# nilsbore/gp_compressor

Hardware: AMD Instinct MI355X
Metric: patches/sec (compress+predict) (higher is better)
Workload: dtype f64; 1 GPU; C2 room scan: 8192 patches x 256 pts per GPU, RBF + Gaussian noise, dense Cholesky fit + predictive mean on the 20x20 grid (m=400); patches_per_gpu=8192, points_per_patch=256, grid_points=400, parallelism=1 GPU, kernel=dense_mfma_w1

## Files before the change

gp_compressor_amd/capi.py:

```python
import ctypes as C
import os
import weakref

import numpy as np

HERE = os.path.dirname(os.path.abspath(__file__))
LIB_PATH = os.environ.get("GPC_LIB_PATH", os.path.join(HERE, "libgpc_hip.so"))

GPC_OK, GPC_EINVAL, GPC_ENOMEM, GPC_ENODEV, GPC_EHIP, GPC_ERANGE = 0, -22, -12, -19, -5, -34
CELL_UNOBSERVED, CELL_OCCUPIED, CELL_FREE = 0, 1, 2
STATUS_OK, STATUS_NOT_SPD, STATUS_NAN, STATUS_SIGMA_CLAMPED, STATUS_OVERFLOW, STATUS_NOT_CONVERGED = 0, 1, 2, 3, 4, 5
MAX_POINTS, MAX_BV = 1024, 256

c_dp = C.POINTER(C.c_double)
c_ip = C.POINTER(C.c_int32)


class Params(C.Structure):
    _fields_ = [("sigmaf_sq", C.c_double), ("l_sq", C.c_double), ("noise", C.c_double), ("eps_tol", C.c_double),
                ("capacity", C.c_int32), ("noise_model", C.c_int32), ("ref_double_noise", C.c_int32),
                ("ref_field_delete_bug", C.c_int32), ("want_variance", C.c_int32), ("reserved", C.c_int32)]


class IrlsParams(C.Structure):
# ... 151 lines not shown
    "gpc_comm_destroy": (None, [_vp]),
    "gpc_comm_world": (C.c_int, [_vp]),
    "gpc_comm_rank": (C.c_int, [_vp]),
    "gpc_comm_library": (C.c_char_p, []),
    "gpc_comm_set_partition": (C.c_int, [_vp, _i, _vp]),
    "gpc_group_start": (C.c_int, []),
    "gpc_group_end": (C.c_int, []),
    "gpc_allgather_fstar_dev": (C.c_int, [_vp, _i, _vp, _vp, _vp]),
    "gpc_unpermute_fstar_dev": (C.c_int, [_vp, _i, _vp, _vp]),
    "gpc_test_exp_host": (None, [_vp, _vp, _i]),
    "gpc_test_exp_small_host": (None, [_vp, _vp, _i]),
    "gpc_test_quantize_host": (C.c_int, [_vp, _i, _i, _vp, _vp, _vp]),
    "gpc_test_rate_allocate_host": (C.c_int, [_i, _i, _vp, _vp, _vp, _vp, _d, _vp, _i, C.c_int64, _i, _vp, _vp, _vp, _vp]),
    "gpc_test_par_memcpy": (None, [_vp, _vp, C.c_size_t]),
    "gpc_test_dense_route": (C.c_int, [_i] * 11 + [_vp, _i, _vp]),
}

_lib = None


def load():
    global _lib
    if _lib is not None:
        return _lib
    try:
        import torch
    except ImportError:
        pass
    if not os.path.exists(LIB_PATH):
        raise GpcError(GPC_ENODEV, f"{LIB_PATH} not built: run `python -c 'import __graft_entry__ as g; g.build()'` "
# ... 1261 lines not shown
    R, ld = a[2].shape
    k = np.zeros(R, dtype=np.int32)
    tg = None if count is None else np.zeros(R, dtype=np.int32)
    res = np.zeros(1, dtype=RATE_RESULT_DTYPE)
    rc = load().gpc_test_rate_allocate_host(R, ld, _ptr(a[0]), _ptr(a[1]), _ptr(a[2]), _ptr(a[3]), float(w_all), _ptr(a[4]), int(unit_all),
                                            int(need), int(bool(refine)), _ptr(a[5]), _ptr(k), _ptr(tg), _ptr(res))
    if rc != GPC_OK:
        raise GpcError(rc, "gpc_test_rate_allocate_host")
    return (k, rate_result(res)) if count is None else (k, tg, rate_result(res))


test_rate_allocate_host.__test__ = False


ROUTE_KINDS = {-1: "no route", 0: "nothing", 1: "one-wave", 2: "register", 3: "tiled", 4: "generic", 5: "split"}
ROUTE_SHAPE = ("w1_npad", "w1_slots", "nt", "export_factor", "waves", "npad", "per_cu", "nt17", "need_big")


def dense_route(P, n_max, n_total=None, ny=1, m=16, variance=False, pointwise=False, alpha_out=False, num_cus=256, irls=False,
                w1_refused=False):
    name = C.create_string_buffer(96)
    shape = np.zeros(len(ROUTE_SHAPE), dtype=np.int32)
    kind = load().gpc_test_dense_route(P, n_max, P * n_max if n_total is None else n_total, ny, m, int(variance), int(pointwise),
                                       int(alpha_out), num_cus, int(irls), int(w1_refused), name, len(name), _ptr(shape))
    return ROUTE_KINDS[kind], name.value.decode(), dict(zip(ROUTE_SHAPE, shape.tolist()))
```

gp_compressor_amd/csrc/dense_api.hip:

```cpp
#include "dense_internal.h"

int dense_check(gpc_ctx* ctx, const gpc_params* prm, int P, const void* off, int n_max, int n_total,
                const void* x0, const void* x1, const void* y, int ny, int m, const void* f_star)
{
    if (!ctx || ctx->dead.load()) return GPC_EINVAL;
    if (!prm) return gpc_fail(ctx, GPC_EINVAL, "params is NULL");
    if (P < 0 || m < 0 || n_total < 0 || n_max < 0) return gpc_fail(ctx, GPC_EINVAL, "negative size");
    if (ny != 1 && ny != 3) return gpc_fail(ctx, GPC_EINVAL, "ny must be 1 (depth) or 3 (RGB), got %d", ny);
    if (P > 0 && !off) return gpc_fail(ctx, GPC_EINVAL, "off is NULL");
    if (n_total > 0 && (!x0 || !x1 || !y)) return gpc_fail(ctx, GPC_EINVAL, "x0/x1/y is NULL");
    if (P > 0 && m > 0 && !f_star) return gpc_fail(ctx, GPC_EINVAL, "f_star is NULL");
    if (n_max > GPC_MAX_POINTS) return gpc_fail(ctx, GPC_ERANGE, "n_max %d > GPC_MAX_POINTS %d", n_max, GPC_MAX_POINTS);
    if (!(prm->l_sq > 0.0) || !(prm->sigmaf_sq >= 0.0) || !(prm->noise >= 0.0))
        return gpc_fail(ctx, GPC_EINVAL, "kernel/noise parameters out of range");
    return GPC_OK;
}

DenseArgs dense_args(const gpc_params* prm, int P, const int32_t* off, int n_max, int n_total, const double* x0, const double* x1,
                     const double* y, int ny, int m, double* f_star, double* alpha_out, int32_t* status)
{
    DenseArgs a{};
    a.prm = *prm;
    a.P = P; a.n_max = n_max; a.n_total = n_total; a.ny = ny; a.m = m;
    a.off = off; a.x0 = x0; a.x1 = x1; a.y = y;
// ... 83 lines not shown

int dense_dispatch(gpc_ctx* ctx, DenseArgs& a, const DenseSite& site, unsigned* seen_gen)
{
    const DenseSwitches sw = dense_switches_read();
    const DenseFacts facts = dense_facts(ctx, a);
    DenseRoute route = dense_route(facts, sw);
    if (route.kind == DENSE_NOTHING) return GPC_OK;
    if (a.n_max < 1) a.n_max = 1;
    if (seen_gen)
        if (int rco = gpc_pipe_chunk_order(ctx, site.stream, seen_gen)) return rco;
    GPC_HIP(ctx, hipSetDevice(ctx->device));
    if (!a.prm.want_variance) a.v_star = nullptr;
    if (int rcp = gpc_debug_poison_lds(ctx, site)) return rcp;
    int grid = 0, rc = GPC_OK;
    if (route.kind == DENSE_ONE_WAVE) {
        for (int cap_w1 = site.w1_cap;;) {
            rc = gpc_ws_reserve(ctx, site, al256(dense_w1_ws_bytes(facts, route, &grid, cap_w1)));
            if (rc != GPC_ENOMEM) break;
            cap_w1 = grid / 2;
            if (cap_w1 < 4 * ctx->num_cus) break;
        }
        if (rc == GPC_ENOMEM) {
            route = dense_route(facts, sw, true);
            if (route.kind == DENSE_NO_ROUTE) return rc;
            (void)hipGetLastError();
        } else if (rc != GPC_OK) {
            return rc;
        }
    }
    switch (route.kind) {
        case DENSE_ONE_WAVE:
            rc = dense_w1_launch(ctx, site, a, route, grid);
            break;
        case DENSE_REGISTER:
            rc = dense_mfma_launch(ctx, site, a, route);
            break;
        case DENSE_TILED:
            if ((rc = gpc_ws_reserve(ctx, site, al256(dense_big_ws_bytes(ctx, a, route, &grid)))) == GPC_OK)
                rc = dense_big_launch(ctx, site, a, route, grid);
            break;
        case DENSE_SPLIT:
            rc = dense_split(ctx, a, site, route, sw.no_hint);
            break;
// ... 13 lines not shown
    *w1_cap = 0;
    const DenseFacts facts = dense_facts(ctx, a);
    const DenseRoute route = dense_route(facts, dense_switches_read());
    int grid = 0, rc = GPC_ENOMEM;
    switch (route.kind) {
        case DENSE_NOTHING:
            return gpc_ws_reserve(ctx, site, front);
        case DENSE_ONE_WAVE:
            for (int cap_w1 = 0;;) {
                rc = gpc_ws_reserve(ctx, site, front + al256(dense_w1_ws_bytes(facts, route, &grid, cap_w1)));
                *w1_cap = cap_w1;
                if (rc != GPC_ENOMEM) break;
                cap_w1 = grid / 2;
                if (cap_w1 < 4 * ctx->num_cus) break;
            }
            return rc;
        case DENSE_REGISTER:
            return gpc_ws_reserve(ctx, site, front + dense_mfma_ws_bytes(a, route));
        case DENSE_TILED:
            return gpc_ws_reserve(ctx, site, front + al256(dense_big_ws_bytes(ctx, a, route, &grid)));
        case DENSE_GENERIC:
            return gpc_ws_reserve(ctx, site, front + dense_generic_ws_bytes(ctx, a, &grid));
        case DENSE_NO_ROUTE:
            return gpc_fail(ctx, GPC_ENOMEM, "no kernel computes the variance of this batch without the one-wave workspace");
        default:
            return gpc_fail(ctx, GPC_EINVAL, "dense_reserve: not a batch of the variance route");
    }
}

extern "C" {
// ... 22 lines not shown
    if (rc != GPC_OK) return rc;
    DenseArgs a = dense_args(params, P, off, n_max, n_total, x0, x1, y, ny, sz * sz, f_star, alpha_out, status);
    a.prm.want_variance = 0;
    a.grid_res = res; a.grid_sz = sz;
    std::lock_guard<std::mutex> lk(ctx->mu);
    return dense_dispatch(ctx, a, dense_site_of(ctx));
}

int gpc_test_dense_route(int P, int n_max, int n_total, int ny, int m, int variance, int pointwise, int alpha_out, int num_cus, int irls,
                         int w1_refused, char* name, int name_cap, int32_t* shape)
{
    const DenseFacts f{P, n_max, n_total, ny, m, variance != 0, pointwise != 0, alpha_out != 0, num_cus, irls != 0};
    const DenseRoute r = dense_route(f, dense_switches_read(), w1_refused != 0);
    if (name && name_cap > 0) snprintf(name, (size_t)name_cap, "%s", r.name);
    if (shape) {
        const int32_t v[GPC_TEST_ROUTE_SHAPE] = {r.w1_npad, r.w1_slots, r.nt, r.export_factor, r.waves, r.npad, r.per_cu, r.nt17, r.need_big};
        memcpy(shape, v, sizeof(v));
    }
    return (int)r.kind;
}

}
```

gp_compressor_amd/csrc/dense_mfma_w1.hip:

```cpp
#include <cstdio>
#include <cstdlib>
#include <type_traits>

#include "gpc_device.h"
#include "dense_internal.h"
#include "mfma_tile.h"

#define W1_NPAD_MAX 512
#define W1_C 4
#define W1_NDT 10
#define W1_NT_OF(npad) ((npad) / 16)
#define W1_TRI_OF(npad) (W1_NT_OF(npad) * (W1_NT_OF(npad) + 1) / 2)
#define W1_TILE(i, j) (((size_t)(i) * (size_t)((i) + 1) / 2 + (size_t)(j)) * MF_IMG)
#define W1_PACK_OF(npad) ((npad) <= 256)
#define W1_LNV_OF(npad) (W1_PACK_OF(npad) ? W1_NT_OF(npad) / 2 : W1_NT_OF(npad))


struct W1Params {
    DenseArgs a;
    double c_exp;
    double pivot_tol;
    double cs, noise_u, sfp, a_out;
    double* ws;
    double* linvt;
    int export_factor;
    unsigned long long* stamps;
};
#define W1_NPH 12
#ifdef W1_STAMPS
#define W1_STAMP(ph)                                                                                                 \
    do {                                                                                                             \
        __builtin_amdgcn_sched_barrier(0);                                                                           \
        const unsigned long long t_now_ = __builtin_amdgcn_s_memtime();                                              \
        st_acc_[ph] += t_now_ - t_prev_;                                                                             \
        t_prev_ = t_now_;                                                                                            \
        __builtin_amdgcn_sched_barrier(0);                                                                           \
    } while (0)
#else
#define W1_STAMP(ph) do { } while (0)
#endif
// ... 29 lines not shown
__device__ static __forceinline__ d4 w1_mfma4_neg(d4 a, d4 b, d4 acc)
{
#pragma unroll
    for (int s = 0; s < 4; ++s) acc = __builtin_amdgcn_mfma_f64_16x16x4f64(a[s], b[s], acc, 0, 0, 1);
    return acc;
}
__device__ static __forceinline__ d4 w1_trsm(d4 lv, d4 src)
{
    const d4 z4 = d4{0.0, 0.0, 0.0, 0.0};
    d4 D = __builtin_amdgcn_mfma_f64_16x16x4f64(lv[0], src[0], z4, 0, 0, 0);
    D = __builtin_amdgcn_mfma_f64_16x16x4f64(lv[1], src[1], D, 0, 0, 0);
    D = __builtin_amdgcn_mfma_f64_16x16x4f64(lv[2], src[2], D, 0, 0, 0);
    return __builtin_amdgcn_mfma_f64_16x16x4f64(lv[3], src[3], D, 0, 0, 0);
}

template <int MODE, int CNT, bool DIAG>
__device__ static __forceinline__ void w1_gram_row(d4 (&v)[W1_C], const double* px0, const double* px1, const double* T, double sf, bool scale_sf,
                                                   double cexp, double noise, bool dbl, int n, int r, int c0, int lr, int lg)
{
    const int pi = MF_TS * r + lr;
    const double xi0 = px0[pi], xi1 = px1[pi];
#pragma unroll
    for (int t = 0; t < CNT; ++t) {
#pragma unroll
        for (int q = 0; q < 4; ++q) {
            const int pj = MF_TS * (c0 + t) + lg + 4 * q;
            const double d0 = xi0 - px0[pj], d1 = xi1 - px1[pj];
            const double sq = __builtin_fma(d0, d0, d1 * d1);
            v[t][q] = MODE == 0 ? gpc_exp_neg(cexp * sq, T) : gpc_expm_poly<MODE == 1 ? 7 : 5>(sq);
        }
// ... 23 lines not shown
        }
    }
}

template <int W1_NPAD>
__global__ __launch_bounds__(64, 2) void dense_w1_kernel(W1Params g)
{
    constexpr int W1_NT = W1_NT_OF(W1_NPAD), W1_TRI = W1_TRI_OF(W1_NPAD);
    __shared__ __attribute__((aligned(16))) double T[GPC_EXP_TABLE_SIZE];
    __shared__ __attribute__((aligned(16))) double px0[W1_NPAD], px1[W1_NPAD], zv[W1_NPAD];
    __shared__ __attribute__((aligned(16))) double rsbuf[32], wsc[32];
    __shared__ __attribute__((aligned(16))) double LinvC[W1_C * MF_IMG];
    constexpr bool W1_PACK = W1_PACK_OF(W1_NPAD);
    constexpr int W1_LNV = W1_LNV_OF(W1_NPAD);
    __shared__ __attribute__((aligned(16))) double dgl[W1_PACK ? W1_LNV * MF_TS : 2];

    const DenseArgs& A = g.a;
    int lane = threadIdx.x;
    int lr = lane & 15, lg = lane >> 4;
#define W1_FRESH_LANE()                                                                                              \
    do {                                                                                                             \
        lane = mf_opaque(lane);                                                                                      \
        lr = lane & 15;                                                                                              \
        lg = lane >> 4;                                                                                              \
    } while (0)
    const int m = A.m;
    const double sf = A.prm.sigmaf_sq, cexp = g.c_exp;
    const bool dbl = A.prm.ref_double_noise != 0;
    const int patch = blockIdx.x;
    double* Lt = g.ws + (size_t)patch * W1_TRI * MF_IMG;
    double* LinvTg = g.linvt + (size_t)patch * W1_LNV * MF_IMG;

    gpc_exp_table_init(T);
    {
        const int o = __builtin_amdgcn_readfirstlane(A.off[patch]);
        const int n = __builtin_amdgcn_readfirstlane(A.off[patch + 1]) - o;
        double* fs = A.f_star + (size_t)patch * m;
        __syncthreads();
        if (n <= 0 || n > W1_NPAD) {
            for (int p = lane; p < m; p += 64) fs[p] = (n == 0) ? 0.0 : __builtin_nan("");
            if (lane == 0 && A.status) A.status[patch] = (n == 0) ? GPC_STATUS_OK : GPC_STATUS_NAN;
            return;
        }
        const int nt = __builtin_amdgcn_readfirstlane((n + MF_TS - 1) / MF_TS);
#ifdef W1_STAMPS
        unsigned long long st_acc_[W1_NPH] = {};
        unsigned long long t_prev_ = __builtin_amdgcn_s_memtime();
#endif

        const double xo0 = A.x0[o], xo1 = A.x1[o];
        double qr0[W1_NPAD / 64], qr1[W1_NPAD / 64];
        double mn0 = xo0, mx0 = xo0, mn1 = xo1, mx1 = xo1;
#pragma unroll
        for (int u = 0; u < W1_NPAD / 64; ++u) {
            const int i = lane + 64 * u;
            const bool live = i < n;
// ... 327 lines not shown
                    }
                    W1_STAMP(7);
                }
            }
            __syncthreads();
            W1_STAMP(8);
        }
#undef W1_BLOCK_INIT
#undef W1_BLOCK_ROW

        if (bad) {
            for (int p = lane; p < m; p += 64) fs[p] = __builtin_nan("");
            if (A.alpha_out)
                for (int i = lane; i < n; i += 64) A.alpha_out[o + i] = __builtin_nan("");
            if (lane == 0 && A.status) A.status[patch] = GPC_STATUS_NOT_SPD;
            return;
        }

        if constexpr (W1_PACK) {
            W1_FRESH_LANE();
            constexpr int NP = W1_NT;
            constexpr int SLEN = NP * NP / 2;
            const int nte = (nt + 1) & ~1, kls = (nt - 1) & ~(W1_C - 1);
            d4 win[W1_BW];
            auto stream_addr = [&](auto P) __attribute__((always_inline)) -> const double* {
                constexpr int q = decltype(P)::value;
                constexpr int pp = w1_pstream_pair(q), i = q - 2 * pp * pp;
                if constexpr (i == 2 * pp) {
                    const int k = nte - 1 - 2 * pp;
                    return (k >= 1 && k - 1 < kls) ? LinvTg + (size_t)(k >> 1) * MF_IMG : Lt;
// ... 63 lines not shown
            };
            w1_static_for<0, W1_BW>([&](auto P) __attribute__((always_inline)) {
                constexpr int q = decltype(P)::value;
                win[q] = mf_img_load_nt(stream_addr(P), lane);
            });
            d4 pa = d4{0.0, 0.0, 0.0, 0.0};
            w1_static_for<0, SLEN>([&](auto P) __attribute__((always_inline)) {
                constexpr int q = decltype(P)::value;
                bw_step(P, win[q % W1_BW], pa);
                if constexpr (q + W1_BW < SLEN) {
                    win[q % W1_BW] = mf_img_load_nt(stream_addr(std::integral_constant<int, q + W1_BW>{}), lane);
                }
            });
        }
        W1_STAMP(9);
        double* av = zv;
        if (A.alpha_out)
            for (int i = lane; i < n; i += 64) A.alpha_out[o + i] = av[i] * g.a_out;

        W1_FRESH_LANE();
        if (m <= 0) {
        } else if (A.xs0 == nullptr && A.grid_sz <= 32) {
            const int sz = A.grid_sz;
            const double res = A.grid_res;
            d4 P[2][2];
#pragma unroll
            for (int mt = 0; mt < 2; ++mt)
#pragma unroll
                for (int nl = 0; nl < 2; ++nl) P[mt][nl] = d4{0.0, 0.0, 0.0, 0.0};
            double gqx[2], gqy[2];
// ... 68 lines not shown
                }
                fs[p] = sfp * s_;
            }
        }
        if (lane == 0 && A.status) A.status[patch] = GPC_STATUS_OK;
#ifdef W1_STAMPS
        W1_STAMP(10);
        if (g.stamps && lane == 0)
            for (int q_ = 0; q_ < W1_NPH; ++q_) atomicAdd(g.stamps + q_, st_acc_[q_]);
#endif
    }
}

static_assert(W1_NPAD_MAX == 512, "dense_route (dense_route.h) names the instances: 256 and 512 points");

size_t dense_w1_ws_bytes(const DenseFacts& f, const DenseRoute& r, int* grid_out, int cap_in)
{
    const int cap = cap_in > 0 && cap_in < r.w1_slots ? cap_in : r.w1_slots;
    const int grid = f.P < cap ? f.P : cap;
    if (grid_out) *grid_out = grid;
    const int npad = r.w1_npad;
    return sizeof(double) * ((size_t)(W1_TRI_OF(npad) + W1_LNV_OF(npad)) * MF_IMG * (size_t)grid + (f.variance ? (size_t)f.n_total : 0));
}

int dense_w1_launch(gpc_ctx* ctx, const DenseSite& site, const DenseArgs& a_in, const DenseRoute& r, int grid)
{
    DenseArgs a = a_in;
    double* v_star = a.v_star;
    double* log_ev = a.log_ev;
    a.v_star = nullptr;
    a.log_ev = nullptr;
    const bool exported = v_star || log_ev;
    W1Params g;
    g.c_exp = (double)(-0.5f) / a.prm.l_sq;
    g.ws = reinterpret_cast<double*>(dense_ws(ctx, site));
    const int npad = r.w1_npad;
    g.linvt = g.ws + (size_t)W1_TRI_OF(npad) * MF_IMG * (size_t)grid;
    g.export_factor = exported ? 1 : 0;
    const double sf = a.prm.sigmaf_sq;
    const bool unit = !exported;
    g.cs = sqrt(-g.c_exp);
    g.noise_u = unit ? a.prm.noise / sf : a.prm.noise;
    g.pivot_tol = GPC_PIVOT_RTOL * (unit ? 1.0 + a.prm.noise / sf : sf + a.prm.noise);
    g.sfp = unit ? 1.0 : sf;
    g.a_out = unit ? 1.0 / sf : 1.0;
    g.stamps = nullptr;
    if (exported) {
        if (v_star) a.m = 0;
        if (!a.alpha_out) a.alpha_out = g.linvt + (size_t)W1_LNV_OF(npad) * MF_IMG * (size_t)grid;
    }
#ifdef W1_STAMPS
    if (getenv("GPC_W1_STAMPS")) {
        GPC_HIP(ctx, hipMalloc(&g.stamps, sizeof(unsigned long long) * W1_NPH));
        GPC_HIP(ctx, hipMemsetAsync(g.stamps, 0, sizeof(unsigned long long) * W1_NPH, site.stream));
    }
#endif
    for (int base = 0; base < a.P; base += grid) {
        const int cnt = a.P - base < grid ? a.P - base : grid;
        g.a = a;
        g.a.P = cnt;
        g.a.off = a.off + base;
        g.a.f_star = a.f_star ? a.f_star + (size_t)base * a.ny * a_in.m : nullptr;
        g.a.status = a.status ? a.status + base : nullptr;
        if (npad == 256) hipLaunchKernelGGL((dense_w1_kernel<256>), dim3(cnt), dim3(64), 0, site.stream, g);
        else hipLaunchKernelGGL((dense_w1_kernel<W1_NPAD_MAX>), dim3(cnt), dim3(64), 0, site.stream, g);
        GPC_HIP(ctx, hipGetLastError());
        if (v_star) {
            DenseArgs av = g.a;
            av.m = a_in.m;
            const int rc = dense_variance_launch(ctx, site, av, W1_NT_OF(256), r.var_w4, g.ws, a.alpha_out, v_star + (size_t)base * a_in.m);
            if (rc != GPC_OK) return rc;
        }
        if (log_ev) {
            const int rc = dense_gauss_evidence_launch(ctx, site, g.a, W1_NT_OF(256), 0, g.ws, 0, a.alpha_out, log_ev + (size_t)base * a.ny);
            if (rc != GPC_OK) return rc;
        }
    }
#ifdef W1_STAMPS
    if (g.stamps) {
        unsigned long long h[W1_NPH];
// ... 14 lines not shown
```

gp_compressor_amd/csrc/dense_route.h:

```cpp
#pragma once

#include <cstdlib>

#include "../../include/gpc.h"

struct DenseSwitches {
    bool force_generic, force_big;
    bool no_w1, no_w1_512, w2;
    bool w1_min_p_set;
    int w1_min_p;
    int w1_slots;
    bool no_split, no_nt17, no_hint;
    bool big_no_w2, big_no_w4;
    int var_w4;
    bool host_no_pipeline, host_one_stream;
};

static inline DenseSwitches dense_switches_read()
{
    DenseSwitches s{};
    s.force_generic = getenv("GPC_FORCE_GENERIC") != nullptr;
    s.force_big = getenv("GPC_FORCE_BIG") != nullptr;
    s.no_w1 = getenv("GPC_NO_W1") != nullptr;
    s.no_w1_512 = getenv("GPC_NO_W1_512") != nullptr;
    s.w2 = getenv("GPC_W2") != nullptr;
    const char* mp = getenv("GPC_W1_MIN_P");
    s.w1_min_p_set = mp != nullptr;
    s.w1_min_p = mp ? atoi(mp) : 0;
    const char* sl = getenv("GPC_W1_SLOTS");
    s.w1_slots = sl && atoi(sl) > 0 ? atoi(sl) : 0;
    s.no_split = getenv("GPC_NO_SPLIT") != nullptr;
    s.no_nt17 = getenv("GPC_NO_NT17") != nullptr;
    s.no_hint = getenv("GPC_NO_HINT") != nullptr;
    s.big_no_w2 = getenv("GPC_BIG_NO_W2") != nullptr;
    s.big_no_w4 = getenv("GPC_BIG_NO_W4") != nullptr;
    const char* vw = getenv("GPC_VAR_W4");
    s.var_w4 = vw ? (atoi(vw) != 0 ? 1 : 0) : -1;
    s.host_no_pipeline = getenv("GPC_HOST_NO_PIPELINE") != nullptr;
    s.host_one_stream = getenv("GPC_HOST_ONE_STREAM") != nullptr;
    return s;
}

struct DenseFacts {
    int P, n_max, n_total, ny, m;
    bool variance;
// ... 7 lines not shown
    DENSE_NO_ROUTE = -1,
    DENSE_NOTHING = 0,
    DENSE_ONE_WAVE,
    DENSE_REGISTER,
    DENSE_TILED,
    DENSE_GENERIC,
    DENSE_SPLIT
};

#define DENSE_W1_MAX_SLOTS 8192

struct DenseRoute {
    DenseKind kind;
    const char* name;
    int w1_npad, w1_slots;
    int nt;
    bool export_factor;
    int waves, npad, per_cu;
    bool nt17, need_big;
    int var_w4;
};

static inline DenseRoute dense_route_register(int n_max, bool variance, int var_w4)
{
    static const char* const names[2][5] = {
        {"dense_mfma_nt4", "dense_mfma_nt8", "dense_mfma_nt12", "dense_mfma_nt16", "dense_mfma_nt17"},
        {"dense_mfma_nt4 + dense_variance", "dense_mfma_nt8 + dense_variance", "dense_mfma_nt12 + dense_variance",
         "dense_mfma_nt16 + dense_variance", ""}};
    const int i = n_max <= 64 ? 0 : n_max <= 128 ? 1 : n_max <= 192 ? 2 : n_max <= 256 ? 3 : 4;
    DenseRoute r{};
    r.kind = DENSE_REGISTER;
    r.nt = i < 4 ? 4 * (i + 1) : 17;
    r.export_factor = variance;
    r.name = names[variance][i];
    r.var_w4 = var_w4;
    return r;
// ... 40 lines not shown
    if (f.P == 0 || (!f.irls && f.m == 0 && !f.alpha_out)) return none;
    if (f.n_max < 1) f.n_max = 1;
    if (f.irls) return dense_route_tiled(f, s);
    const int n = f.n_max;
    const bool v = f.variance, depth = f.ny == 1, ny_ok = f.ny == 1 || f.ny == 3;
    if (!s.force_generic && !s.force_big && ny_ok) {
        const bool no_split = f.P == 1 || s.no_split;
        const int min_p = s.w1_min_p_set ? s.w1_min_p : 4 * f.num_cus;
        const bool w1_can = depth && (v ? n <= 256 && n > 192 && f.pointwise : n <= 512);
        if (w1_can && f.P >= min_p && f.P > 1 && !s.no_w1 && !(n > 256 && s.no_w1_512)) {
            if (!w1_refused) {
                DenseRoute r{};
                r.kind = DENSE_ONE_WAVE;
                r.w1_npad = n <= 256 ? 256 : 512;
                r.w1_slots = s.w1_slots ? s.w1_slots : DENSE_W1_MAX_SLOTS;
                r.var_w4 = s.var_w4;
                r.name = v ? "dense_mfma_w1 + dense_variance" : n <= 256 ? "dense_mfma_w1" : "dense_mfma_w1_512";
                return r;
            }
            if (v) { none.kind = DENSE_NO_ROUTE; return none; }
        }
        if (n > 192 && n <= 256 && depth && !v && f.P > 1 && s.w2) return dense_route_tiled(f, s);
        if (n <= 256 || (no_split && n <= 17 * 16 && depth && !v && !s.no_nt17)) return dense_route_register(n, v, s.var_w4);
        const bool uniform = (long long)f.P * n == (long long)f.n_total;
        if (!v && n <= GPC_MAX_POINTS && !no_split && !(uniform && n > 17 * 16)) {
            DenseRoute r = dense_route_tiled(f, s);
            r.kind = DENSE_SPLIT;
            r.nt17 = depth && !s.no_nt17;
            r.need_big = !(r.nt17 && n <= 17 * 16);
            r.name = !r.need_big ? "dense_mfma_nt16 + dense_mfma_nt17" : r.nt17 ? "dense_mfma_nt16 + dense_mfma_nt17 + dense_mfma_big"
// ... 12 lines not shown
```

gp_compressor_amd/csrc/gpc_api.hip:

```cpp
#include <algorithm>
#include <cstdlib>
#include <numeric>
#include <vector>

#include "gpc_device.h"
#include "dense_internal.h"

extern "C" {

int gpc_version(void) { return GPC_VERSION; }

void gpc_default_params_dense(gpc_params* p)
{
    if (!p) return;
    std::memset(p, 0, sizeof(*p));
    p->sigmaf_sq = 0.05 * 0.05;
    p->l_sq = 3.0 * 3.0;
    p->noise = 0.04 * 0.04;
    p->eps_tol = 0.0;
    p->capacity = 0;
    p->noise_model = 0;
    p->ref_double_noise = 1;
    p->ref_field_delete_bug = 1;
    p->want_variance = 0;
// ... 181 lines not shown
    if (lds_words[(threadIdx.x * 17) % words] == 0ull) lds_words[0] = 1ull;
}

}

int gpc_debug_poison_lds(gpc_ctx* ctx, const DenseSite& site)
{
    const bool on = getenv("GPC_POISON_LDS") != nullptr;
    if (!on || !ctx) return GPC_OK;
    GPC_HIP(ctx, hipFuncSetAttribute(reinterpret_cast<const void*>(gpc_poison_lds_kernel), hipFuncAttributeMaxDynamicSharedMemorySize,
                                     160 * 1024));
    const int bytes = 160 * 1024;
    hipLaunchKernelGGL(gpc_poison_lds_kernel, dim3(ctx->num_cus * 2), dim3(256), bytes, site.stream, bytes / 8);
    GPC_HIP(ctx, hipGetLastError());
    if (const size_t len = ctx->ws ? dense_ws_len(ctx, site) : 0) GPC_HIP(ctx, hipMemsetAsync(dense_ws(ctx, site), 0xFF, len, site.stream));
    return GPC_OK;
}

extern "C" {

int gpc_debug_poison_lds(gpc_ctx* ctx)
{
    return ctx ? gpc_debug_poison_lds(ctx, dense_site_of(ctx)) : GPC_OK;
}


__global__ void gpc_noise_eval_kernel(int model, double s20, int n, const double* y, const double* x, const double* sx, double* q, double* r)
{
    const int i = blockIdx.x * blockDim.x + threadIdx.x;
    if (i >= n) return;
// ... 93 lines not shown
```

gp_compressor_amd/csrc/gpc_internal.h:

```cpp
#pragma once

#include <hip/hip_runtime.h>

#include <cstdarg>
#include <cstdlib>
#include <cstdint>
#include <cstdio>
#include <cstring>
#include <atomic>
#include <mutex>
#include <string>
#include <utility>
#include <vector>

#include "../../include/gpc.h"

#define GPC_PIVOT_RTOL 1e-14

struct gpc_ctx {
    int device = 0;
    hipStream_t own_stream = nullptr;
    hipStream_t stream = nullptr;
    int num_cus = 256;
    void* ws = nullptr;
    size_t ws_bytes = 0;
    int32_t* tickets = nullptr;
    void* io = nullptr;
    size_t io_bytes = 0;
    void* pin_in = nullptr;
    size_t pin_in_bytes = 0;
    void* pin_out = nullptr;
    size_t pin_out_bytes = 0;
    hipStream_t s_in = nullptr, s_out = nullptr, s_c2 = nullptr;
    bool pipe_active = false;
    unsigned foreign_gen = 0;
    hipEvent_t ev[3][16] = {};
    std::mutex host_mu;
    const int32_t* hint_off = nullptr;
    int hint_P = 0, hint_le256 = 0, hint_le272 = 0;
    std::mutex mu;
// ... 138 lines not shown
        if (rc != GPC_OK) return rc;
        if (err != hipSuccess) return gpc_fail(ctx, err == hipErrorOutOfMemory ? GPC_ENOMEM : GPC_EHIP, "%s: %s", entry, hipGetErrorString(err));
        return GPC_OK;
    }
};

static inline int gpc_ws_reserve(gpc_ctx* ctx, hipStream_t stream, bool pipe_chunk, size_t bytes)
{
    if (ctx->pipe_active && !pipe_chunk && !getenv("GPC_NO_PIPE_ORDER")) {
        ++ctx->foreign_gen;
        GPC_HIP(ctx, hipEventRecord(ctx->ev[0][GPC_EV_PIPE_ORDER], ctx->own_stream));
        GPC_HIP(ctx, hipEventRecord(ctx->ev[1][GPC_EV_PIPE_ORDER], ctx->s_c2));
        GPC_HIP(ctx, hipStreamWaitEvent(stream, ctx->ev[0][GPC_EV_PIPE_ORDER], 0));
        GPC_HIP(ctx, hipStreamWaitEvent(stream, ctx->ev[1][GPC_EV_PIPE_ORDER], 0));
    }
    if (bytes <= ctx->ws_bytes) return GPC_OK;
    void* nw = nullptr;
    const char* lim = getenv("GPC_WS_FAIL_ABOVE");
    if (lim && bytes > (size_t)atoll(lim)) return gpc_fail(ctx, GPC_ENOMEM, "workspace allocation failed (GPC_WS_FAIL_ABOVE)");
    hipError_t e = hipMalloc(&nw, bytes);
    if (e != hipSuccess) {
        (void)hipGetLastError();
        if (!ctx->ws) return gpc_fail(ctx, GPC_ENOMEM, "workspace allocation failed");
        GPC_HIP(ctx, hipStreamSynchronize(stream));
        const size_t old_bytes = ctx->ws_bytes;
        GPC_HIP(ctx, hipFree(ctx->ws));
        ctx->ws = nullptr;
        ctx->ws_bytes = 0;
        e = hipMalloc(&nw, bytes);
        if (e != hipSuccess) {
// ... 32 lines not shown
```

include/gpc.h:

```cpp
#ifndef GPC_H
#define GPC_H

#include <stddef.h>
#include <stdint.h>

#ifdef __cplusplus
extern "C" {
#endif

#define GPC_VERSION 100

#define GPC_OK 0
#define GPC_EINVAL (-22)
#define GPC_ENOMEM (-12)
#define GPC_ENODEV (-19)
#define GPC_EHIP (-5)
#define GPC_ERANGE (-34)

#define GPC_STATUS_OK 0
#define GPC_STATUS_NOT_SPD 1
#define GPC_STATUS_NAN 2
#define GPC_STATUS_SIGMA_CLAMPED 3
#define GPC_STATUS_OVERFLOW 4
#define GPC_STATUS_NOT_CONVERGED 5
// ... 304 lines not shown
int gpc_comm_rank(const gpc_comm* c);
const char* gpc_comm_library(void);
int gpc_comm_set_partition(gpc_comm* c, int P, const int32_t* slot_patch);
int gpc_group_start(void);
int gpc_group_end(void);
int gpc_allgather_fstar_dev(gpc_comm* c, int row_doubles, const double* local_f, double* gathered, double* f_star);
int gpc_unpermute_fstar_dev(gpc_comm* c, int row_doubles, const double* gathered, double* f_star);

void gpc_test_exp_host(const double* x, double* out, int n);
void gpc_test_exp_small_host(const double* x, double* out, int n);
int gpc_test_quantize_host(const double* v, int b, int w, uint16_t* q, float* range, double* deq);
int gpc_test_rate_allocate_host(int R, int ld, const int32_t* kmax, const double* d0, const double* d, const double* w, double w_all,
                                const int32_t* unit, int unit_all, int64_t need, int refine, const int32_t* count, int32_t* k, int32_t* target,
                                gpc_rate_result* result);
void gpc_test_par_memcpy(void* dst, const void* src, size_t bytes);
#define GPC_TEST_ROUTE_SHAPE 9
int gpc_test_dense_route(int P, int n_max, int n_total, int ny, int m, int variance, int pointwise, int alpha_out, int num_cus,
                         int irls, int w1_refused, char* name, int name_cap, int32_t* shape);

#ifdef __cplusplus
}
#endif
#endif
```

Before: 5.601 million patches/s.

## Pool one-wave Cholesky workspace slots across resident workgroups via per-XCD rings

New measurement: 5.563 million patches/s. Within noise of the previous version (-0.7%).

```diff
diff --git a/gp_compressor_amd/capi.py b/gp_compressor_amd/capi.py
--- a/gp_compressor_amd/capi.py
+++ b/gp_compressor_amd/capi.py
@@ -189,6 +189,7 @@
     "gpc_test_rate_allocate_host": (C.c_int, [_i, _i, _vp, _vp, _vp, _vp, _d, _vp, _i, C.c_int64, _i, _vp, _vp, _vp, _vp]),
     "gpc_test_par_memcpy": (None, [_vp, _vp, C.c_size_t]),
     "gpc_test_dense_route": (C.c_int, [_i] * 11 + [_vp, _i, _vp]),
+    "gpc_test_dense_w1_ws": (C.c_int, [_i] * 8 + [_vp]),
 }
 
 _lib = None
@@ -1480,7 +1481,7 @@
 
 
 ROUTE_KINDS = {-1: "no route", 0: "nothing", 1: "one-wave", 2: "register", 3: "tiled", 4: "generic", 5: "split"}
-ROUTE_SHAPE = ("w1_npad", "w1_slots", "nt", "export_factor", "waves", "npad", "per_cu", "nt17", "need_big")
+ROUTE_SHAPE = ("w1_npad", "w1_slots", "nt", "export_factor", "waves", "npad", "per_cu", "nt17", "need_big", "w1_pooled", "w1_resident")
 
 
 def dense_route(P, n_max, n_total=None, ny=1, m=16, variance=False, pointwise=False, alpha_out=False, num_cus=256, irls=False,
@@ -1490,3 +1491,12 @@
     kind = load().gpc_test_dense_route(P, n_max, P * n_max if n_total is None else n_total, ny, m, int(variance), int(pointwise),
                                        int(alpha_out), num_cus, int(irls), int(w1_refused), name, len(name), _ptr(shape))
     return ROUTE_KINDS[kind], name.value.decode(), dict(zip(ROUTE_SHAPE, shape.tolist()))
+
+
+def dense_w1_ws(P, n_max, resident, shards=8, n_total=None, variance=False, pointwise=False, num_cus=256):
+    out = np.zeros(5, dtype=np.int64)
+    rc = load().gpc_test_dense_w1_ws(P, n_max, P * n_max if n_total is None else n_total, int(variance), int(pointwise), num_cus, resident,
+                                     shards, _ptr(out))
+    if rc < 0:
+        return None, None
+    return bool(rc), dict(zip(("bytes", "slots", "slot_bytes", "pool_bytes", "per_shard"), out.tolist()))
diff --git a/gp_compressor_amd/csrc/dense_api.hip b/gp_compressor_amd/csrc/dense_api.hip
--- a/gp_compressor_amd/csrc/dense_api.hip
+++ b/gp_compressor_amd/csrc/dense_api.hip
@@ -121,9 +121,13 @@
     if (int rcp = gpc_debug_poison_lds(ctx, site)) return rcp;
     int grid = 0, rc = GPC_OK;
     if (route.kind == DENSE_ONE_WAVE) {
+        bool refused = false;
         for (int cap_w1 = site.w1_cap;;) {
             rc = gpc_ws_reserve(ctx, site, al256(dense_w1_ws_bytes(facts, route, &grid, cap_w1)));
             if (rc != GPC_ENOMEM) break;
+            refused = true;
+            route.w1_pooled = false;
+            route.w1_resident = 0;
             cap_w1 = grid / 2;
             if (cap_w1 < 4 * ctx->num_cus) break;
         }
@@ -134,6 +138,7 @@
         } else if (rc != GPC_OK) {
             return rc;
         }
+        if (refused) ctx->err[0] = 0;
     }
     switch (route.kind) {
         case DENSE_ONE_WAVE:
@@ -177,6 +182,7 @@
                 cap_w1 = grid / 2;
                 if (cap_w1 < 4 * ctx->num_cus) break;
             }
+            if (rc == GPC_OK && *w1_cap > 0) ctx->err[0] = 0;
             return rc;
         case DENSE_REGISTER:
             return gpc_ws_reserve(ctx, site, front + dense_mfma_ws_bytes(a, route));
@@ -229,10 +235,28 @@
     const DenseRoute r = dense_route(f, dense_switches_read(), w1_refused != 0);
     if (name && name_cap > 0) snprintf(name, (size_t)name_cap, "%s", r.name);
     if (shape) {
-        const int32_t v[GPC_TEST_ROUTE_SHAPE] = {r.w1_npad, r.w1_slots, r.nt, r.export_factor, r.waves, r.npad, r.per_cu, r.nt17, r.need_big};
+        const int32_t v[GPC_TEST_ROUTE_SHAPE] = {r.w1_npad, r.w1_slots, r.nt, r.export_factor, r.waves, r.npad, r.per_cu, r.nt17, r.need_big,
+                                                 r.w1_pooled, r.w1_resident};
         memcpy(shape, v, sizeof(v));
     }
     return (int)r.kind;
 }
 
-}
+int gpc_test_dense_w1_ws(int P, int n_max, int n_total, int variance, int pointwise, int num_cus, int resident, int shards, int64_t* out)
+{
+    const DenseFacts f{P, n_max, n_total, 1, 16, variance != 0, pointwise != 0, false, num_cus, false};
+    const DenseRoute r = dense_route(f, dense_switches_read());
+    if (r.kind != DENSE_ONE_WAVE) return -1;
+    int slots = 0, per_shard = 0;
+    const size_t bytes = dense_w1_ws_sized(f, r, resident, shards, 0, &slots, &per_shard);
+    if (out) {
+        out[0] = (int64_t)bytes;
+        out[1] = slots;
+        out[2] = (int64_t)(sizeof(double) * dense_w1_slot_doubles(r.w1_npad));
+        out[3] = per_shard ? (int64_t)dense_w1_pool_bytes(slots) : 0;
+        out[4] = per_shard;
+    }
+    return r.w1_pooled ? 1 : 0;
+}
+
+}
diff --git a/gp_compressor_amd/csrc/dense_mfma_w1.hip b/gp_compressor_amd/csrc/dense_mfma_w1.hip
--- a/gp_compressor_amd/csrc/dense_mfma_w1.hip
+++ b/gp_compressor_amd/csrc/dense_mfma_w1.hip
@@ -1,5 +1,7 @@
 #include <cstdio>
+#include <climits>
 #include <cstdlib>
+#include <mutex>
 #include <type_traits>
 
 #include "gpc_device.h"
@@ -24,6 +26,8 @@
     double* ws;
     double* linvt;
     int export_factor;
+    unsigned long long* pool;
+    int pool_n, pool_shards;
     unsigned long long* stamps;
 };
 #define W1_NPH 12
@@ -83,6 +87,58 @@
     return __builtin_amdgcn_mfma_f64_16x16x4f64(lv[3], src[3], D, 0, 0, 0);
 }
 
+#define W1_POOL_TRIES 4096
+__device__ static __forceinline__ int w1_pool_shard(int shards)
+{
+    return (int)(__builtin_amdgcn_s_getreg(20 | (0 << 6) | (3 << 11)) % (unsigned)shards);
+}
+__device__ static __forceinline__ int w1_pool_pop(unsigned long long* pool, int pool_n, int shards, int lane)
+{
+    const int sh = w1_pool_shard(shards);
+    unsigned e = 0xFFFFu;
+    if (lane == 0) {
+        const unsigned long long t = atomicAdd(pool + DENSE_W1_POOL_HEAD(sh), 1ull);
+        const unsigned long long* ent = pool + DENSE_W1_POOL_RING + (size_t)sh * pool_n + (size_t)(t % (unsigned long long)pool_n);
+        for (int tries = 0; tries < W1_POOL_TRIES; ++tries) {
+            const unsigned long long v = __hip_atomic_load(ent, __ATOMIC_RELAXED, __HIP_MEMORY_SCOPE_AGENT);
+            if ((v >> 16) == t) {
+                e = (unsigned)(v & 0xFFFFu);
+                break;
+            }
+            __builtin_amdgcn_s_sleep(8);
+        }
+    }
+    const int slot = __builtin_amdgcn_readfirstlane((int)e);
+    return slot >= sh * pool_n && slot < (sh + 1) * pool_n ? slot : -1;
+}
+__device__ static __forceinline__ void w1_pool_stash(unsigned long long* stash, unsigned long long* pool, int pool_n, int shards, int slot,
+                                                     int lane)
+{
+    if (lane == 0) {
+        stash[0] = reinterpret_cast<unsigned long long>(pool);
+        stash[1] = ((unsigned long long)(unsigned)shards << 32) | ((unsigned long long)(unsigned)pool_n << 16) | (unsigned long long)(slot & 0xFFFF);
+    }
+}
+__device__ static __forceinline__ void w1_pool_push(const unsigned long long* stash, int lane)
+{
+    unsigned long long* const pool = reinterpret_cast<unsigned long long*>(stash[0]);
+    if (pool == nullptr) return;
+    asm volatile("s_waitcnt vmcnt(0)" ::: "memory");
+    if (lane == 0) {
+        const unsigned long long sn = stash[1], pool_n = (sn >> 16) & 0xFFFFull, slot = sn & 0xFFFFull;
+        const int sh = w1_pool_shard((int)(sn >> 32));
+        const unsigned long long j = atomicAdd(pool + DENSE_W1_POOL_TAIL(sh), 1ull);
+        __hip_atomic_store(pool + DENSE_W1_POOL_RING + (size_t)sh * pool_n + (size_t)(j % pool_n), ((j + pool_n) << 16) | slot,
+                           __ATOMIC_RELAXED, __HIP_MEMORY_SCOPE_AGENT);
+    }
+}
+__global__ void w1_pool_init_kernel(unsigned long long* pool, int pool_n, int shards)
+{
+    const int i = blockIdx.x * blockDim.x + threadIdx.x;
+    if (i < DENSE_W1_POOL_RING) pool[i] = 0;
+    if (i < pool_n * shards) pool[DENSE_W1_POOL_RING + i] = ((unsigned long long)(i % pool_n) << 16) | (unsigned long long)i;
+}
+
 template <int MODE, int CNT, bool DIAG>
 __device__ static __forceinline__ void w1_gram_row(d4 (&v)[W1_C], const double* px0, const double* px1, const double* T, double sf, bool scale_sf,
                                                    double cexp, double noise, bool dbl, int n, int r, int c0, int lr, int lg)
@@ -136,6 +192,7 @@
     constexpr bool W1_PACK = W1_PACK_OF(W1_NPAD);
     constexpr int W1_LNV = W1_LNV_OF(W1_NPAD);
     __shared__ __attribute__((aligned(16))) double dgl[W1_PACK ? W1_LNV * MF_TS : 2];
+    unsigned long long* const stash = reinterpret_cast<unsigned long long*>(wsc + 30);
 
     const DenseArgs& A = g.a;
     int lane = threadIdx.x;
@@ -150,8 +207,10 @@
     const double sf = A.prm.sigmaf_sq, cexp = g.c_exp;
     const bool dbl = A.prm.ref_double_noise != 0;
     const int patch = blockIdx.x;
-    double* Lt = g.ws + (size_t)patch * W1_TRI * MF_IMG;
-    double* LinvTg = g.linvt + (size_t)patch * W1_LNV * MF_IMG;
+    const int slot = g.pool ? w1_pool_pop(g.pool, g.pool_n, g.pool_shards, lane) : patch;
+    w1_pool_stash(stash, slot >= 0 ? g.pool : nullptr, g.pool_n, g.pool_shards, slot, lane);
+    double* Lt = g.ws + (size_t)max(slot, 0) * W1_TRI * MF_IMG;
+    double* LinvTg = g.linvt + (size_t)max(slot, 0) * W1_LNV * MF_IMG;
 
     gpc_exp_table_init(T);
     {
@@ -159,9 +218,10 @@
         const int n = __builtin_amdgcn_readfirstlane(A.off[patch + 1]) - o;
         double* fs = A.f_star + (size_t)patch * m;
         __syncthreads();
-        if (n <= 0 || n > W1_NPAD) {
+        if (n <= 0 || n > W1_NPAD || slot < 0) {
             for (int p = lane; p < m; p += 64) fs[p] = (n == 0) ? 0.0 : __builtin_nan("");
             if (lane == 0 && A.status) A.status[patch] = (n == 0) ? GPC_STATUS_OK : GPC_STATUS_NAN;
+            w1_pool_push(stash, lane);
             return;
         }
         const int nt = __builtin_amdgcn_readfirstlane((n + MF_TS - 1) / MF_TS);
@@ -519,6 +579,7 @@
             if (A.alpha_out)
                 for (int i = lane; i < n; i += 64) A.alpha_out[o + i] = __builtin_nan("");
             if (lane == 0 && A.status) A.status[patch] = GPC_STATUS_NOT_SPD;
+            w1_pool_push(stash, lane);
             return;
         }
 
@@ -612,6 +673,7 @@
             });
         }
         W1_STAMP(9);
+        w1_pool_push(stash, lane);
         double* av = zv;
         if (A.alpha_out)
             for (int i = lane; i < n; i += 64) A.alpha_out[o + i] = av[i] * g.a_out;
@@ -710,13 +772,65 @@
 
 static_assert(W1_NPAD_MAX == 512, "dense_route (dense_route.h) names the instances: 256 and 512 points");
 
+static_assert(sizeof(double) * MF_IMG == 2048, "dense_route.h sizes the workspace of this kernel");
+
+struct W1Residency { int dyn_lds, per_cu, xcds; };
+static W1Residency dense_w1_residency(int npad, int want)
+{
+    static std::mutex mu;
+    static struct { int dev, npad, want; W1Residency res; } cache[16];
+    static int cached = 0;
+    int dev = 0;
+    if (hipGetDevice(&dev) != hipSuccess) return {0, 0, 1};
+    std::lock_guard<std::mutex> lk(mu);
+    for (int i = 0; i < cached; ++i)
+        if (cache[i].dev == dev && cache[i].npad == npad && cache[i].want == want) return cache[i].res;
+    const void* fn = npad == 256 ? reinterpret_cast<const void*>(dense_w1_kernel<256>) : reinterpret_cast<const void*>(dense_w1_kernel<W1_NPAD_MAX>);
+    auto ask = [&](int dyn) {
+        int occ = 0;
+        const hipError_t e = npad == 256 ? hipOccupancyMaxActiveBlocksPerMultiprocessor(&occ, dense_w1_kernel<256>, 64, (size_t)dyn)
+                                         : hipOccupancyMaxActiveBlocksPerMultiprocessor(&occ, dense_w1_kernel<W1_NPAD_MAX>, 64, (size_t)dyn);
+        if (e != hipSuccess) (void)hipGetLastError();
+        return e == hipSuccess && occ > 0 ? occ : 0;
+    };
+    W1Residency res{0, ask(0), 1};
+    if (res.per_cu > want) {
+        hipFuncAttributes fa;
+        int lds_cu = 0;
+        if (hipFuncGetAttributes(&fa, fn) != hipSuccess || hipDeviceGetAttribute(&lds_cu, hipDeviceAttributeMaxSharedMemoryPerMultiprocessor, dev) != hipSuccess ||
+            lds_cu <= 0) {
+            (void)hipGetLastError();
+            res.per_cu = 0;
+        } else {
+            const int total = ((lds_cu / (want + 1) + lds_cu / want) / 2) & ~255;
+            res.dyn_lds = total > (int)fa.sharedSizeBytes ? total - (int)fa.sharedSizeBytes : 0;
+            res.per_cu = ask(res.dyn_lds);
+            while (res.per_cu > want && res.dyn_lds + (int)fa.sharedSizeBytes + 1024 <= 64 * 1024) res.per_cu = ask(res.dyn_lds += 1024);
+            if (res.per_cu > want) res = {0, 0, 1};
+        }
+    }
+    if (hipDeviceGetAttribute(&res.xcds, hipDeviceAttributeNumberOfXccs, dev) != hipSuccess || res.xcds < 1 || res.xcds > DENSE_W1_POOL_SHARDS_MAX) {
+        (void)hipGetLastError();
+        res = {res.dyn_lds, 0, 1};
+    }
+    if (cached < 16) cache[cached++] = {dev, npad, want, res};
+    return res;
+}
+static int dense_w1_resident_wgs(const DenseRoute& r, int num_cus, int* shards, int* dyn_lds)
+{
+    const W1Residency res = dense_w1_residency(r.w1_npad, r.w1_resident);
+    if (dyn_lds) *dyn_lds = res.dyn_lds;
+    *shards = res.xcds;
+    return res.per_cu > 0 && num_cus > 0 ? res.per_cu * ((num_cus + res.xcds - 1) / res.xcds) * res.xcds : INT_MAX;
+}
+
 size_t dense_w1_ws_bytes(const DenseFacts& f, const DenseRoute& r, int* grid_out, int cap_in)
 {
-    const int cap = cap_in > 0 && cap_in < r.w1_slots ? cap_in : r.w1_slots;
-    const int grid = f.P < cap ? f.P : cap;
-    if (grid_out) *grid_out = grid;
-    const int npad = r.w1_npad;
-    return sizeof(double) * ((size_t)(W1_TRI_OF(npad) + W1_LNV_OF(npad)) * MF_IMG * (size_t)grid + (f.variance ? (size_t)f.n_total : 0));
+    static_assert(dense_w1_slot_doubles_c(256) == (size_t)(W1_TRI_OF(256) + W1_LNV_OF(256)) * MF_IMG &&
+                  dense_w1_slot_doubles_c(512) == (size_t)(W1_TRI_OF(512) + W1_LNV_OF(512)) * MF_IMG, "the slot of dense_route.h is this kernel's");
+    int shards = 1;
+    const int resident = r.w1_pooled ? dense_w1_resident_wgs(r, f.num_cus, &shards, nullptr) : 0;
+    return dense_w1_ws_sized(f, r, resident, shards, cap_in, grid_out);
 }
 
 int dense_w1_launch(gpc_ctx* ctx, const DenseSite& site, const DenseArgs& a_in, const DenseRoute& r, int grid)
@@ -741,6 +855,30 @@
     g.sfp = unit ? 1.0 : sf;
     g.a_out = unit ? 1.0 / sf : 1.0;
     g.stamps = nullptr;
+    g.pool = nullptr;
+    g.pool_n = 0;
+    g.pool_shards = 1;
+    int dyn_lds = 0;
+    if (r.w1_pooled) {
+        if (exported) return gpc_fail(ctx, GPC_EINVAL, "dense_w1_launch: the exported factor has one slot per patch");
+        int shards = 1, per_shard = 0;
+        if (grid != dense_w1_pool_slots(a.P, dense_w1_resident_wgs(r, ctx->num_cus, &shards, &dyn_lds), shards, &per_shard))
+            return gpc_fail(ctx, GPC_EINVAL, "dense_w1_launch: %d slots for a pooled launch of %d patches", grid, a.P);
+        if (per_shard) {
+            g.pool = reinterpret_cast<unsigned long long*>(g.linvt + (size_t)W1_LNV_OF(npad) * MF_IMG * (size_t)grid);
+            g.pool_n = per_shard;
+            g.pool_shards = shards;
+            if (ctx->w1_pool_at != g.pool || ctx->w1_pool_n != grid || ctx->w1_pool_gen + 1 != ctx->ws_gen) {
+                const int cnt = grid > DENSE_W1_POOL_RING ? grid : DENSE_W1_POOL_RING;
+                hipLaunchKernelGGL(w1_pool_init_kernel, dim3((cnt + 255) / 256), dim3(256), 0, site.stream, g.pool, per_shard, shards);
+                GPC_HIP(ctx, hipGetLastError());
+            }
+            ctx->w1_pool_at = g.pool;
+            ctx->w1_pool_n = grid;
+            ctx->w1_pool_gen = ctx->ws_gen;
+        }
+    }
+    const int per_launch = r.w1_pooled ? a.P : grid;
     if (exported) {
         if (v_star) a.m = 0;
         if (!a.alpha_out) a.alpha_out = g.linvt + (size_t)W1_LNV_OF(npad) * MF_IMG * (size_t)grid;
@@ -751,15 +889,15 @@
         GPC_HIP(ctx, hipMemsetAsync(g.stamps, 0, sizeof(unsigned long long) * W1_NPH, site.stream));
     }
 #endif
-    for (int base = 0; base < a.P; base += grid) {
-        const int cnt = a.P - base < grid ? a.P - base : grid;
+    for (int base = 0; base < a.P; base += per_launch) {
+        const int cnt = a.P - base < per_launch ? a.P - base : per_launch;
         g.a = a;
         g.a.P = cnt;
         g.a.off = a.off + base;
         g.a.f_star = a.f_star ? a.f_star + (size_t)base * a.ny * a_in.m : nullptr;
         g.a.status = a.status ? a.status + base : nullptr;
-        if (npad == 256) hipLaunchKernelGGL((dense_w1_kernel<256>), dim3(cnt), dim3(64), 0, site.stream, g);
-        else hipLaunchKernelGGL((dense_w1_kernel<W1_NPAD_MAX>), dim3(cnt), dim3(64), 0, site.stream, g);
+        if (npad == 256) hipLaunchKernelGGL((dense_w1_kernel<256>), dim3(cnt), dim3(64), dyn_lds, site.stream, g);
+        else hipLaunchKernelGGL((dense_w1_kernel<W1_NPAD_MAX>), dim3(cnt), dim3(64), dyn_lds, site.stream, g);
         GPC_HIP(ctx, hipGetLastError());
         if (v_star) {
             DenseArgs av = g.a;
diff --git a/gp_compressor_amd/csrc/dense_route.h b/gp_compressor_amd/csrc/dense_route.h
--- a/gp_compressor_amd/csrc/dense_route.h
+++ b/gp_compressor_amd/csrc/dense_route.h
@@ -1,5 +1,7 @@
 #pragma once
 
+#include <cassert>
+#include <cstddef>
 #include <cstdlib>
 
 #include "../../include/gpc.h"
@@ -10,11 +12,22 @@
     bool w1_min_p_set;
     int w1_min_p;
     int w1_slots;
+    int w1_resident;
+    bool w1_no_pool;
     bool no_split, no_nt17, no_hint;
     bool big_no_w2, big_no_w4;
     int var_w4;
     bool host_no_pipeline, host_one_stream;
 };
+
+#define DENSE_W1_RESIDENT_MIN 5
+#define DENSE_W1_RESIDENT_MAX 8
+#define DENSE_W1_RESIDENT_256 8
+#define DENSE_W1_RESIDENT_512 7
+static inline int dense_w1_resident_clamp(int r)
+{
+    return r < DENSE_W1_RESIDENT_MIN ? DENSE_W1_RESIDENT_MIN : r > DENSE_W1_RESIDENT_MAX ? DENSE_W1_RESIDENT_MAX : r;
+}
 
 static inline DenseSwitches dense_switches_read()
 {
@@ -29,6 +42,9 @@
     s.w1_min_p = mp ? atoi(mp) : 0;
     const char* sl = getenv("GPC_W1_SLOTS");
     s.w1_slots = sl && atoi(sl) > 0 ? atoi(sl) : 0;
+    const char* rs = getenv("GPC_W1_RESIDENT");
+    s.w1_resident = rs ? dense_w1_resident_clamp(atoi(rs)) : 0;
+    s.w1_no_pool = getenv("GPC_W1_NO_POOL") != nullptr;
     s.no_split = getenv("GPC_NO_SPLIT") != nullptr;
     s.no_nt17 = getenv("GPC_NO_NT17") != nullptr;
     s.no_hint = getenv("GPC_NO_HINT") != nullptr;
@@ -66,12 +82,53 @@
     DenseKind kind;
     const char* name;
     int w1_npad, w1_slots;
+    bool w1_pooled;
+    int w1_resident;
     int nt;
     bool export_factor;
     int waves, npad, per_cu;
     bool nt17, need_big;
     int var_w4;
 };
+
+constexpr size_t dense_w1_slot_doubles_c(int npad)
+{
+    return ((size_t)(npad / 16) * (size_t)(npad / 16 + 1) / 2 + (size_t)(npad <= 256 ? npad / 32 : npad / 16)) * 256;
+}
+static inline size_t dense_w1_slot_doubles(int npad) { return dense_w1_slot_doubles_c(npad); }
+#define DENSE_W1_POOL_SHARDS_MAX 16
+#define DENSE_W1_POOL_HEAD(shard) (32 * (shard))
+#define DENSE_W1_POOL_TAIL(shard) (32 * (shard) + 16)
+#define DENSE_W1_POOL_RING (32 * DENSE_W1_POOL_SHARDS_MAX)
+#define DENSE_W1_POOL_MAX_SLOTS 65535
+static inline size_t dense_w1_pool_bytes(int slots) { return 8 * ((size_t)DENSE_W1_POOL_RING + (size_t)slots); }
+static inline int dense_w1_pool_slots(int P, int resident, int shards, int* per_shard)
+{
+    const int ns = shards < 1 ? 1 : shards > DENSE_W1_POOL_SHARDS_MAX ? DENSE_W1_POOL_SHARDS_MAX : shards;
+    const long long each = ((long long)resident + ns - 1) / ns, all = each * ns;
+    const bool pool = P > all && all <= DENSE_W1_POOL_MAX_SLOTS;
+    const int slots = pool ? (int)all : P;
+    assert(slots >= 0 && (slots >= P || slots >= resident));
+    if (per_shard) *per_shard = pool ? (int)each : 0;
+    return slots;
+}
+static inline size_t dense_w1_ws_sized(const DenseFacts& f, const DenseRoute& r, int resident, int shards, int cap_in, int* slots_out,
+                                       int* per_shard_out = nullptr)
+{
+    int slots, per_shard = 0;
+    size_t tail;
+    if (r.w1_pooled) {
+        slots = dense_w1_pool_slots(f.P, resident, shards, &per_shard);
+        tail = per_shard ? dense_w1_pool_bytes(slots) : 0;
+    } else {
+        const int cap = cap_in > 0 && cap_in < r.w1_slots ? cap_in : r.w1_slots;
+        slots = f.P < cap ? f.P : cap;
+        tail = f.variance ? sizeof(double) * (size_t)f.n_total : 0;
+    }
+    if (slots_out) *slots_out = slots;
+    if (per_shard_out) *per_shard_out = per_shard;
+    return sizeof(double) * dense_w1_slot_doubles(r.w1_npad) * (size_t)slots + tail;
+}
 
 static inline DenseRoute dense_route_register(int n_max, bool variance, int var_w4)
 {
@@ -142,6 +199,8 @@
                 r.kind = DENSE_ONE_WAVE;
                 r.w1_npad = n <= 256 ? 256 : 512;
                 r.w1_slots = s.w1_slots ? s.w1_slots : DENSE_W1_MAX_SLOTS;
+                r.w1_pooled = !v && !s.w1_no_pool;
+                r.w1_resident = !r.w1_pooled ? 0 : s.w1_resident ? s.w1_resident : n <= 256 ? DENSE_W1_RESIDENT_256 : DENSE_W1_RESIDENT_512;
                 r.var_w4 = s.var_w4;
                 r.name = v ? "dense_mfma_w1 + dense_variance" : n <= 256 ? "dense_mfma_w1" : "dense_mfma_w1_512";
                 return r;
diff --git a/gp_compressor_amd/csrc/gpc_api.hip b/gp_compressor_amd/csrc/gpc_api.hip
--- a/gp_compressor_amd/csrc/gpc_api.hip
+++ b/gp_compressor_amd/csrc/gpc_api.hip
@@ -219,6 +219,7 @@
     hipLaunchKernelGGL(gpc_poison_lds_kernel, dim3(ctx->num_cus * 2), dim3(256), bytes, site.stream, bytes / 8);
     GPC_HIP(ctx, hipGetLastError());
     if (const size_t len = ctx->ws ? dense_ws_len(ctx, site) : 0) GPC_HIP(ctx, hipMemsetAsync(dense_ws(ctx, site), 0xFF, len, site.stream));
+    ++ctx->ws_gen;
     return GPC_OK;
 }
 
diff --git a/gp_compressor_amd/csrc/gpc_internal.h b/gp_compressor_amd/csrc/gpc_internal.h
--- a/gp_compressor_amd/csrc/gpc_internal.h
+++ b/gp_compressor_amd/csrc/gpc_internal.h
@@ -24,6 +24,10 @@
     int num_cus = 256;
     void* ws = nullptr;
     size_t ws_bytes = 0;
+    unsigned ws_gen = 0;
+    const void* w1_pool_at = nullptr;
+    int w1_pool_n = 0;
+    unsigned w1_pool_gen = 0;
     int32_t* tickets = nullptr;
     void* io = nullptr;
     size_t io_bytes = 0;
@@ -192,6 +196,7 @@
         GPC_HIP(ctx, hipStreamWaitEvent(stream, ctx->ev[0][GPC_EV_PIPE_ORDER], 0));
         GPC_HIP(ctx, hipStreamWaitEvent(stream, ctx->ev[1][GPC_EV_PIPE_ORDER], 0));
     }
+    ++ctx->ws_gen;
     if (bytes <= ctx->ws_bytes) return GPC_OK;
     void* nw = nullptr;
     const char* lim = getenv("GPC_WS_FAIL_ABOVE");
diff --git a/include/gpc.h b/include/gpc.h
--- a/include/gpc.h
+++ b/include/gpc.h
@@ -342,9 +342,10 @@
                                 const int32_t* unit, int unit_all, int64_t need, int refine, const int32_t* count, int32_t* k, int32_t* target,
                                 gpc_rate_result* result);
 void gpc_test_par_memcpy(void* dst, const void* src, size_t bytes);
-#define GPC_TEST_ROUTE_SHAPE 9
+#define GPC_TEST_ROUTE_SHAPE 11
 int gpc_test_dense_route(int P, int n_max, int n_total, int ny, int m, int variance, int pointwise, int alpha_out, int num_cus,
                          int irls, int w1_refused, char* name, int name_cap, int32_t* shape);
+int gpc_test_dense_w1_ws(int P, int n_max, int n_total, int variance, int pointwise, int num_cus, int resident, int shards, int64_t* out);
 
 #ifdef __cplusplus
 }
```
